# tuanad121/Python-WORLD

Measured on AMD Instinct MI355X. Metric: analysis+synthesis frames/sec (and xRT), 16 kHz / 5 ms hop, higher is better.
Workload: dtype f64; 1 GPU; BASELINE config 2 per GPU: 64 x 10 s synthetic 16 kHz utterances, DIO+StoneMask+CheapTrick+D4C encode + pulse-wise synthesis decode with on-device Philox noise (not the reference-parity host-noise path), HBM-resident; utterances_per_gpu=64, distinct_utterances=64, fs=16000, lanes_per_gpu=1

## Files before the change

python-world_amd/csrc/wh_minphase.h:

```cpp
#pragma once
#include <type_traits>
#include "wh_fft.h"

namespace {

constexpr int ft_syn(int n) { return n >= 2048 ? 512 : 256; }

__device__ __attribute__((noinline)) double4 cis_pair_call(double a0, double b0, double a1, double b1) {
  const double e0 = exp(a0), e1 = exp(a1);
  double s0, c0, s1, c1;
  sincospi(b0, &s0, &c0);
  sincospi(b1, &s1, &c1);
  return make_double4(e0 * c0, e0 * s0, e1 * c1, e1 * s1);
}
__device__ __attribute__((noinline)) double4 cis_pair_tab_call(double a0, double b0, double a1, double b1, wh::ckp<const double2> tw256,
                                                               wh::ckp<const double> mt) {
  const double2 sc0 = wh::tsincospi(b0, tw256), sc1 = wh::tsincospi(b1, tw256);
  const double e0 = wh::texp(a0, mt), e1 = wh::texp(a1, mt);
  return make_double4(e0 * sc0.y, e0 * sc0.x, e1 * sc1.y, e1 * sc1.x);
}
__device__ __attribute__((noinline)) double2 log_pair_call(double x, double y) { return make_double2(wh::flog(x), wh::flog(y)); }
__device__ __attribute__((noinline)) double log_call(double x) { return wh::flog(x); }

template <int M, bool INV, int GT, int FT, bool WAVE>
__device__ __forceinline__ void mp_fft(wh::ckp<double2> zb, wh::ckp<const double2> tw) {
  if constexpr (WAVE) wh::fft_lds_wave<M, INV, GT, FT>(zb, tw);
  else wh::fft_lds<M, INV, GT, FT>(zb, tw);
}
struct SpectrumIdentity {
  __device__ __forceinline__ double2 operator()(int, double2 e) const { return e; }
};
struct NoSide {};
template <int N, int GT, bool WAVE = false, bool TAB = false, class Mul = SpectrumIdentity, class Side = NoSide>
__device__ __forceinline__ void min_phase_response(wh::ckp<double2> zb, wh::ckp<const double2> tw_base, wh::ckp<const double> mt, double delay_pi, Mul mul = Mul(),
                                                   Side side = Side()) {
#pragma clang fp contract(fast)
  constexpr int FT = ft_syn(N);
  constexpr int M = N / 2;
  constexpr int PP = (M / 2 + 1 + GT - 1) / GT;
  const wh::ckp<double> zr = wh::ck_as<double>(zb);
  const int gt = WH_TID & (GT - 1);
  const wh::ckp<const double2> WH_RESTRICT w = tw_base + N;
  if constexpr (WAVE && !std::is_same<Side, NoSide>::value) wh::fft_lds_wave<M, false, GT, FT>(zb, tw_base + M, side);
  else mp_fft<M, false, GT, FT, WAVE>(zb, tw_base + M);
  {
    double ck[PP], cm[PP];
#pragma unroll
    for (int p = 0; p < PP; ++p) {
      const int k = gt + p * GT;
      ck[p] = cm[p] = 0.0;
      if (k <= M / 2) {
        const double2 a = zb[k], b = zb[M - k];
        if (k == 0) {
          ck[p] = a.x + a.y;
          cm[p] = a.x - a.y;
        } else {
          const double er = 0.5 * (a.x + b.x), dr = 0.5 * (a.x - b.x), di = 0.5 * (a.y + b.y);
          const double2 wk = wh::ldg2(w + k);
          const double tr = fma(wk.x, di, wk.y * dr);
          ck[p] = er + tr;
          cm[p] = er - tr;
        }
      }
    }
    wh::sync<FT>();
#pragma unroll
    for (int p = 0; p < PP; ++p) {
      const int k = gt + p * GT;
      if (k <= M / 2) {
        if (k == 0) {
          zr[0] = ck[p];
          zr[M] = 2 * cm[p];
        } else {
          zr[N - k] = 2 * ck[p];
          zr[M + k] = 2 * cm[p];
        }
      }
    }
    for (int n = 1 + gt; n < M; n += GT) zr[n] = 0.0;
    wh::sync<FT>();
  }
  mp_fft<M, false, GT, FT, WAVE>(zb, tw_base + M);
#pragma unroll 1
  for (int k = gt; k <= M / 2; k += GT) {
    const double2 a = zb[k], b = zb[M - k];
    double2 x0, x1;
    const double2 wk = wh::ldg2(w + k);
    if (k == 0) {
      x0 = make_double2(a.x + a.y, 0.0);
      x1 = make_double2(a.x - a.y, 0.0);
    } else {
      const double er = 0.5 * (a.x + b.x), ei = 0.5 * (a.y - b.y);
      const double dr = 0.5 * (a.x - b.x), di = 0.5 * (a.y + b.y);
      const double tr = fma(wk.x, di, wk.y * dr);
      const double ti = fma(wk.y, di, -(wk.x * dr));
      x0 = make_double2(er + tr, ei + ti);
      x1 = make_double2(er - tr, ti - ei);
    }
    const double a0 = x0.x / N, b0 = -x0.y / N * M_1_PI - delay_pi * (double)k;
    const double a1 = x1.x / N, b1 = -x1.y / N * M_1_PI - delay_pi * (double)(M - k);
    double4 cis;
    if constexpr (TAB) cis = cis_pair_tab_call(a0, b0, a1, b1, tw_base + 256, mt);
    else cis = cis_pair_call(a0, b0, a1, b1);
    double2 A = mul(k, make_double2(cis.x, cis.y)), B = mul(M - k, make_double2(cis.z, cis.w));
    if (k == 0) {
      A.y = 0.0;
      B.y = 0.0;
    }
    const double er = A.x + B.x, ei = A.y - B.y;
    const double dr = A.x - B.x, di = A.y + B.y;
    const double orr = fma(dr, wk.x, di * wk.y);
    const double oi = fma(di, wk.x, -(dr * wk.y));
    zb[k] = make_double2(er - oi, ei + orr);
    if (k != 0) zb[M - k] = make_double2(er + oi, orr - ei);
  }
  wh::sync<FT>();
  mp_fft<M, true, GT, FT, WAVE>(zb, tw_base + M);
}

}
```

python-world_amd/csrc/wh_resp_pair.h:

```cpp
#pragma once

namespace {

__device__ __forceinline__ bool resp_pairable(const RespArgs& A, int vuv0, int noise_size0, int vuv1, int noise_size1) {
  const int nd0 = noise_size0 > 3 ? noise_size0 : 3, nd1 = noise_size1 > 3 ? noise_size1 : 3;
  return vuv0 == 0 && vuv1 == 0 && A.noise == nullptr && nd0 + nd1 <= kRespNoise;
}

template <int N>
__device__ __forceinline__ void response_pair(const RespArgs& A, const PulseRec& r0, const PulseRec& r1, char* smem, wh::ckp<double> ring,
                                              RunState& rs, wh::ckp<double> WH_RESTRICT row) {
#pragma clang fp contract(fast)
  const double* __restrict__ spectrogram = A.spectrogram;
  const double2* __restrict__ tw_raw = A.tw_base;
  asm volatile("" : "+s"(tw_raw));
  const wh::ckp<const double2> tw_base = wh::ck_make(tw_raw, WH_TWIDDLE_ENTRIES, wh::WH_CK_TWIDDLE);
  const double* __restrict__ mt_raw = A.math_tab;
  asm volatile("" : "+s"(mt_raw));
  const wh::ckp<const double> mt = wh::ck_make(mt_raw, wh::kMtEntries, wh::WH_CK_TABLE);
  constexpr int FT = ft_syn(N);
  constexpr int K = N / 2 + 1;
  constexpr int NZ = kRespNoise;
  constexpr int R = N / FT;
  constexpr int GT = FT / 2;
  static_assert(GT == 2 * WH_WAVE && R <= 4 && 2 * NZ <= N, "one side wave per chain; the staged noise fits the first chain's buffer");
  using L = RespLds<N>;
  static_assert(NZ == L::kNoiseLen, "the noise block of the layout is the chunk this function stages");
  const wh::ckp<double> lds_all = wh::ck_make(reinterpret_cast<double*>(smem), L::kPulse, wh::WH_CK_LDS_OTHER);
  const wh::ckp<double> zrA = wh::ck_sub(lds_all, L::kChainA, L::kChainLen, wh::WH_CK_LDS_MAIN);
  const wh::ckp<double2> zbA = wh::ck_as<double2>(zrA);
  const wh::ckp<double> zrP = wh::ck_sub(lds_all, L::kChainP, L::kChainLen, wh::WH_CK_LDS_AUX);
  const wh::ckp<double2> zbP = wh::ck_as<double2>(zrP);
  const wh::ckp<double> rap = wh::ck_sub(lds_all, L::kRap, L::kRapLen, wh::WH_CK_LDS_OTHER);
  const wh::ckp<double> nz = wh::ck_sub(lds_all, L::kNoise, L::kNoiseLen, wh::WH_CK_LDS_OTHER);
  const wh::ckp<double> scratch = wh::ck_sub(lds_all, L::kScratch, L::kScratchLen, wh::WH_CK_LDS_SCRATCH);

  RSTAGE_BEGIN
  wh::sync<FT>();
  const int u = r0.u;
  const int64_t ny = A.meta[u].ny;
  RSTAGE_COUNT(kRsNUnvoicedVuv) RSTAGE_COUNT(kRsNUnvoicedVuv) RSTAGE_COUNT(kRsNPairs) RSTAGE_COUNT(kRsNPulses) RSTAGE_COUNT(kRsNPulses)
  {
    const bool same_rows = r0.rows == r1.rows;
    const double* s_lo0 = spectrogram + (r0.rows & 0xffffffffll) * K;
    const double* s_hi0 = spectrogram + (r0.rows >> 32) * K;
    const double* s_lo1 = spectrogram + (r1.rows & 0xffffffffll) * K;
    const double* s_hi1 = spectrogram + (r1.rows >> 32) * K;
    const bool same0 = r0.weight < 0.0, same1 = r1.weight < 0.0;
    const double b0 = same0 ? 0.0 : r0.weight, b1 = same1 ? 0.0 : r1.weight;
    const double a0 = 1 - b0, a1 = 1 - b1;
    constexpr int KQ = (K + FT - 1) / FT;
    double rl0[KQ], rh0[KQ], rl1[KQ], rh1[KQ];
#pragma unroll
    for (int q = 0; q < KQ; ++q) {
      const int k = WH_TID + q * FT;
      const int kc = k < K ? k : K - 1;
      rl0[q] = s_lo0[kc];
      rh0[q] = s_hi0[kc];
    }
    if (same_rows) {
#pragma unroll
      for (int q = 0; q < KQ; ++q) {
        rl1[q] = rl0[q];
        rh1[q] = rh0[q];
      }
    } else {
#pragma unroll
      for (int q = 0; q < KQ; ++q) {
        const int k = WH_TID + q * FT;
        const int kc = k < K ? k : K - 1;
        rl1[q] = s_lo1[kc];
        rh1[q] = s_hi1[kc];
      }
    }
#pragma unroll
    for (int q = 0; q < KQ; ++q) {
      const int k = WH_TID + q * FT;
      if (k >= K) break;
      double w0 = same0 ? rl0[q] : fma(a0, rl0[q], b0 * rh0[q]);
      double w1 = same1 ? rl1[q] : fma(a1, rl1[q], b1 * rh1[q]);
      if (w0 == 0.0) w0 = 2.220446049250313e-16;
      if (w1 == 0.0) w1 = 2.220446049250313e-16;
      const double2 lg = log_pair_call(fabs(w0), fabs(w1));
      const double l0 = lg.x / 2, l1 = lg.y / 2;
      zrA[k] = l0;
      zrP[k] = l1;
      if (k > 0 && k < N / 2) {
        zrA[N - k] = l0;
        zrP[N - k] = l1;
      }
    }
  }
  RSTAGE_MARK(kRsSetup)
  const int nd0 = r0.noise_size > 3 ? r0.noise_size : 3, nd1 = r1.noise_size > 3 ? r1.noise_size : 3;
  const int64_t noff0 = r0.noff, noff1 = r1.noff;
  const uint64_t seed = A.seed;
  auto noise_side = [&](int i, int) {
    const uint64_t key = philox_key(seed, (uint64_t)u);
    const int lane = i & 63;
    const int p = __builtin_amdgcn_readfirstlane(i - lane) >> 6;
    const int64_t noff = p == 0 ? noff0 : noff1;
    const int nd = p == 0 ? nd0 : nd1, at = p == 0 ? 0 : nd0;
    const int64_t blk0 = noff >> 1, b1 = (noff + nd - 1) >> 1;
    for (int c = 0; blk0 + c <= b1; c += 64) {
      const int64_t blk = blk0 + c + lane;
      double part = 0.0;
      if (blk <= b1) {
        const double2 z = normal_pair(key, (uint64_t)blk);
        const int j = (int)(2 * blk - noff);
        if (j >= 0) {
          part += z.x;
          nz[at + j] = z.x;
        }
        if (j + 1 < nd) {
          part += z.y;
          nz[at + j + 1] = z.y;
        }
      }
      part = wh::wave_sum(part);
      if (lane == 0) scratch[4 * p + (c >> 6)] = part;
    }
  };
  wh::sync<FT>();
  RSTAGE_MARK(kRsNoise)
  {
    const int g = WH_TID / GT;
    min_phase_response<N, GT, true, resp_table_cis<N>()>(g == 0 ? zbA : zbP, tw_base, mt, 0.0, SpectrumIdentity(), noise_side);
  }
  RSTAGE_MARK(kRsChainsPair)
  double mean0, mean1;
  {
    const int nb0 = (int)(((noff0 + nd0 - 1) >> 1) - (noff0 >> 1)) + 1, nb1 = (int)(((noff1 + nd1 - 1) >> 1) - (noff1 >> 1)) + 1;
    double t0 = 0.0, t1 = 0.0;
#pragma unroll
    for (int w = 0; w < (NZ / 2 + 1 + 63) / 64; ++w) {
      if (w * 64 < nb0) t0 += scratch[w];
      if (w * 64 < nb1) t1 += scratch[4 + w];
    }
    mean0 = t0 / (double)nd0;
    mean1 = t1 / (double)nd1;
  }
  for (int n = WH_TID; n < N; n += FT) rap[rap_index(n)] = zrA[(n + N / 2) & (N - 1)] / N;
  wh::sync<FT>();
  for (int j = WH_TID; j < NZ; j += FT) {
    zrA[j] = j < nd0 ? nz[j] - mean0 : 0.0;
    zrA[NZ + j] = j < nd1 ? nz[nd0 + j] - mean1 : 0.0;
  }
  wh::sync<FT>();
  const int m0 = WH_TID * R;
  auto excite_and_add = [&](wh::ckp<double> nzb, int nd, int64_t pidx) {
    double acc[R];
#pragma unroll
    for (int q = 0; q < R; ++q) acc[q] = 0.0;
    noise_conv_groups<R>(rap, nzb, nd, m0, 0, acc);
    const int64_t s1 = pidx - N / 2 + 1;
    ring_advance<N>(ring, rs, row, s1, ny);
#pragma unroll
    for (int q = 0; q < R; ++q) {
      const int mm = m0 + q;
      const int64_t tgt = s1 + mm;
      if (tgt < 1) continue;
      if (tgt < ny) ring[(int)(tgt & (N - 1))] += acc[q];
      else if (mm == N - 1) rs.last += acc[q];
    }
  };
  excite_and_add(zrA, nd0, r0.pidx);
  RSTAGE_MARK(kRsConv)
  wh::sync<FT>();
  for (int n = WH_TID; n < N; n += FT) rap[rap_index(n)] = zrP[(n + N / 2) & (N - 1)] / N;
  wh::sync<FT>();
  excite_and_add(zrA + NZ, nd1, r1.pidx);
  RSTAGE_MARK(kRsOverlapAdd)
}

}
```

python-world_amd/csrc/wh_resp_pulse.h:

```cpp
#pragma once

namespace {

template <int R>
__device__ __forceinline__ void noise_conv_groups(wh::ckp<double> rap, wh::ckp<double> nzb, int cnt, int m0, int64_t j0, double (&acc)[R]) {
#pragma clang fp contract(fast)
  auto load_group = [&](int base, double (&g)[R]) {
#pragma unroll
    for (int t = 0; t < R; t += 2) {
      double2 v = make_double2(0.0, 0.0);
      if (base >= 0) v = wh::ck_as<const double2>(rap + rap_index(base + t))[0];
      g[t] = v.x;
      g[t + 1] = v.y;
    }
  };
  auto block = [&](int j, const double (&hi)[R], const double (&lo)[R]) {
    double n[R];
#pragma unroll
    for (int t = 0; t < R; t += 2) {
      const double2 v = wh::ck_as<const double2>(nzb + (j + t))[0];
      n[t] = v.x;
      n[t + 1] = v.y;
    }
#pragma unroll
    for (int sft = 0; sft < R; ++sft)
#pragma unroll
      for (int q = 0; q < R; ++q) acc[q] = fma(n[sft], q - sft >= 0 ? hi[q - sft] : lo[R + q - sft], acc[q]);
  };
  double ga[R], gb[R];
  const int mb0 = m0 - (int)j0;
  load_group(mb0, ga);
  load_group(mb0 - R, gb);
  const int steps = ((cnt + 2 * R - 1) / (2 * R)) * (2 * R);
  for (int j = 0; j < steps; j += 2 * R) {
    block(j, ga, gb);
    load_group(mb0 - j - 2 * R, ga);
    block(j + R, gb, ga);
    load_group(mb0 - j - 3 * R, gb);
  }
}

template <int N>
__device__ __forceinline__ void response_pulse(const RespArgs& A, const PulseRec& rec, char* smem, wh::ckp<double> ring, RunState& rs,
                                               wh::ckp<double> WH_RESTRICT row,
                                               const double (&dcw)[N / ft_syn(N) <= 4 ? N / ft_syn(N) : 1]) {
#pragma clang fp contract(fast)
  const SynUtt* __restrict__ meta = A.meta;
  const double* __restrict__ spectrogram = A.spectrogram;
  const double* __restrict__ aperiodicity = A.aperiodicity;
  const double fs = A.fs;
  const double* __restrict__ noise = A.noise;
  const uint64_t seed = A.seed;
  const double* __restrict__ dc_base = A.dc_base;
  const double2* __restrict__ tw_raw = A.tw_base;
  asm volatile("" : "+s"(tw_raw));
  const wh::ckp<const double2> tw_base = wh::ck_make(tw_raw, WH_TWIDDLE_ENTRIES, wh::WH_CK_TWIDDLE);
  const double* __restrict__ mt_raw = A.math_tab;
  asm volatile("" : "+s"(mt_raw));
  const wh::ckp<const double> mt = wh::ck_make(mt_raw, wh::kMtEntries, wh::WH_CK_TABLE);
  constexpr int FT = ft_syn(N);
  constexpr int K = N / 2 + 1;
  constexpr int NZ = kRespNoise;
  constexpr int NZC = resp_conv8<N>() ? 252 : NZ;
  constexpr int R = N / FT;
  static_assert(R % 2 == 0 && NZ % (2 * R) == 0, "pairwise reads; whole blocks of 2R noise samples");
  constexpr int GT = FT >= 256 ? FT / 2 : FT;
  constexpr int NG = FT / GT;
  using L = RespLds<N>;
  static_assert(NZ == L::kNoiseLen, "the noise block of the layout is the chunk this function stages");
  const wh::ckp<double> lds_all = wh::ck_make(reinterpret_cast<double*>(smem), L::kPulse, wh::WH_CK_LDS_OTHER);
  const wh::ckp<double> zrA = wh::ck_sub(lds_all, L::kChainA, L::kChainLen, wh::WH_CK_LDS_MAIN);
  const wh::ckp<double2> zbA = wh::ck_as<double2>(zrA);
  const wh::ckp<double> zrP = wh::ck_sub(lds_all, L::kChainP, L::kChainLen, wh::WH_CK_LDS_AUX);
  const wh::ckp<double2> zbP = wh::ck_as<double2>(zrP);
  const wh::ckp<double> rap = wh::ck_sub(lds_all, L::kRap, L::kRapLen, wh::WH_CK_LDS_OTHER);
  const wh::ckp<double> nz = wh::ck_sub(lds_all, L::kNoise, L::kNoiseLen, wh::WH_CK_LDS_OTHER);
  const wh::ckp<double> scratch = wh::ck_sub(lds_all, L::kScratch, L::kScratchLen, wh::WH_CK_LDS_SCRATCH);

  RSTAGE_BEGIN
  wh::sync<FT>();
  const int u = rec.u;
  const SynUtt m = meta[u];
  const int64_t pidx = rec.pidx;
  const double shift = rec.shift;
  const int64_t noise_size = rec.noise_size;

  const int64_t row_lo = rec.rows & 0xffffffffll, row_hi = rec.rows >> 32;
  const double bw = rec.weight;
  const bool same = bw < 0.0;
  const double b = same ? 0.0 : bw;
  const double a = 1 - b;
  const double* s_lo = spectrogram + row_lo * K;
  const double* s_hi = spectrogram + row_hi * K;
  const double* a_lo = aperiodicity + row_lo * K;
  const double* a_hi = aperiodicity + row_hi * K;
  constexpr int KQ = (K + FT - 1) / FT;
  double rsl[KQ], rsh[KQ], ral[KQ], rah[KQ];
  const bool need_ap = rec.vuv != 0;
#pragma unroll
  for (int q = 0; q < KQ; ++q) {
    const int k = WH_TID + q * FT;
    const int kc = k < K ? k : K - 1;
    rsl[q] = s_lo[kc];
    rsh[q] = s_hi[kc];
    if constexpr (resp_skip_ap<N>()) {
      ral[q] = rah[q] = 0.0;
    } else {
      ral[q] = a_lo[kc];
      rah[q] = a_hi[kc];
    }
  }
  double ap0_lo, ap0_hi;
  if constexpr (resp_skip_ap<N>()) {
    ap0_lo = ap0_hi = 0.0;
    if (need_ap) {
#pragma unroll
      for (int q = 0; q < KQ; ++q) {
        const int k = WH_TID + q * FT;
        const int kc = k < K ? k : K - 1;
        ral[q] = a_lo[kc];
        rah[q] = a_hi[kc];
      }
      ap0_lo = a_lo[0];
      ap0_hi = a_hi[0];
    }
  } else {
    ap0_lo = a_lo[0];
    ap0_hi = a_hi[0];
  }
  asm volatile("" : "+v"(ap0_lo), "+v"(ap0_hi));
  double aper0;
  {
    const double al = ap0_lo * ap0_lo, ah = ap0_hi * ap0_hi;
    aper0 = same ? al : a * al + b * ah;
  }
  const bool voiced = (rec.vuv != 0) && (aper0 <= 0.999);
  RSTAGE_COUNT(voiced ? kRsNVoiced : (rec.vuv == 0 ? kRsNUnvoicedVuv : kRsNUnvoicedRows))
  RSTAGE_COUNT(kRsNPulses)
#pragma unroll
  for (int q = 0; q < KQ; ++q) {
    const int k = WH_TID + q * FT;
    if (k >= K) break;
    const double sl = rsl[q], sh = rsh[q];
    double v, w;
    auto spectra = [&]() {
      double al = ral[q] * ral[q], ah = rah[q] * rah[q];
      if constexpr (resp_skip_ap<N>()) asm volatile("" : "+v"(al), "+v"(ah));
      const double pl = fmax(0.001, 1 - al), ph = fmax(0.001, 1 - ah);
      const double sp = same ? sl : a * sl + b * sh;
      const double pe = same ? pl : a * pl + b * ph;
      const double ap = same ? al : a * al + b * ah;
      v = sp * pe;
      if (v == 0.0) v = 2.220446049250313e-16;
      w = voiced ? sp * ap : sp;
    };
    if constexpr (resp_skip_ap<N>()) {
      v = 0.0;
      w = same ? sl : a * sl + b * sh;
      if (voiced) spectra();
    } else {
      spectra();
    }
    if (w == 0.0) w = 2.220446049250313e-16;
    double2 lg;
    if (voiced) lg = log_pair_call(fabs(w), fabs(v));
    else lg = make_double2(log_call(fabs(w)), 0.0);
    const double lw = lg.x / 2;
    zrA[k] = lw;
    if (k > 0 && k < N / 2) zrA[N - k] = lw;
    if (voiced) {
      const double lv = lg.y / 2;
      zrP[k] = lv;
      if (k > 0 && k < N / 2) zrP[N - k] = lv;
    }
  }
  RSTAGE_MARK(kRsSetup)
  const int64_t nd = noise_size > 3 ? noise_size : 3;
  const int64_t noff = rec.noff;
  auto noise_at = [&](int64_t j) -> double {
    if (noise) {
      const int64_t q = noff + j;
      return q < m.noise_len ? noise[m.noise_off + q] : 0.0;
    }
    return normal_at(philox_key(seed, (uint64_t)u), (uint64_t)(noff + j));
  };
  constexpr bool ROLES = resp_wave_fft<N>();
  static_assert(!ROLES || NZ / 2 + 1 <= FT, "a run that fits nz is at most one Philox block per thread");
  const bool side_noise = ROLES && noise == nullptr && nd <= NZ;
  auto noise_side = [&](int i, int n) {
    if (!side_noise) return;
    const uint64_t key = philox_key(seed, (uint64_t)u);
    const int lane = i & 63;
    const int64_t blk0 = noff >> 1, b1 = (noff + nd - 1) >> 1;
    for (int c = __builtin_amdgcn_readfirstlane(i - lane); blk0 + c <= b1; c += n) {
      const int64_t blk = blk0 + c + lane;
      double part = 0.0;
      if (blk <= b1) {
        const double2 z = normal_pair(key, (uint64_t)blk);
        const int64_t j = 2 * blk - noff;
        if (j >= 0) {
          part += z.x;
          nz[j] = z.x;
        }
        if (j + 1 < nd) {
          part += z.y;
          nz[j + 1] = z.y;
        }
      }
      part = wh::wave_sum(part);
      if (lane == 0) scratch[c >> 6] = part;
    }
  };
  double mean = 0.0;
  if (side_noise) {
    wh::sync<FT>();
  } else {
    double part = 0.0;
    if (noise) {
      for (int64_t j = WH_TID; j < nd; j += FT) {
        const double v = noise_at(j);
        part += v;
        if (j < NZ) nz[j] = v;
      }
    } else {
      const uint64_t key = philox_key(seed, (uint64_t)u);
      const int64_t b1 = (noff + nd - 1) >> 1;
      for (int64_t blk = (noff >> 1) + WH_TID; blk <= b1; blk += FT) {
        const double2 z = normal_pair(key, (uint64_t)blk);
        const int64_t j = 2 * blk - noff;
        if (j >= 0) {
          part += z.x;
          if (j < NZ) nz[j] = z.x;
        }
        if (j + 1 < nd) {
          part += z.y;
          if (j + 1 < NZ) nz[j + 1] = z.y;
        }
      }
    }
    mean = wh::block_sum<FT>(part, scratch) / (double)nd;
  }

  RSTAGE_MARK(kRsNoise)
  const double coef_pi = 2.0 * fs / N;
  if constexpr (ROLES) {
    if (NG == 2 && voiced) {
      const int g = WH_TID / GT;
      min_phase_response<N, GT, true, resp_table_cis<N>()>(g == 0 ? zbA : zbP, tw_base, mt, g == 0 ? 0.0 : coef_pi * shift, SpectrumIdentity(), noise_side);
    } else {
      min_phase_response<N, FT, true, resp_table_cis<N>()>(zbA, tw_base, mt, 0.0, SpectrumIdentity(), noise_side);
      if (voiced) min_phase_response<N, FT, true, resp_table_cis<N>()>(zbP, tw_base, mt, coef_pi * shift);
    }
  } else if (NG == 2 && voiced) {
    const int g = WH_TID / GT;
    min_phase_response<N, GT, false, resp_table_cis<N>()>(g == 0 ? zbA : zbP, tw_base, mt, g == 0 ? 0.0 : coef_pi * shift);
  } else {
    min_phase_response<N, FT, false, resp_table_cis<N>()>(zbA, tw_base, mt, 0.0);
    if (voiced) min_phase_response<N, FT, false, resp_table_cis<N>()>(zbP, tw_base, mt, coef_pi * shift);
  }
  RSTAGE_MARK(voiced ? kRsChainsVoiced : kRsChainsUnvoiced)
  if (side_noise) {
    const int n_blk = (int)(((noff + nd - 1) >> 1) - (noff >> 1)) + 1;
    double t = 0.0;
#pragma unroll
    for (int w = 0; w < (NZ / 2 + 1 + 63) / 64; ++w)
      if (w * 64 < n_blk) t += scratch[w];
    mean = t / (double)nd;
  }
  for (int n = WH_TID; n < N; n += FT) rap[rap_index(n)] = zrA[(n + N / 2) & (N - 1)] / N;
  wh::sync<FT>();

  double acc[R];
#pragma unroll
  for (int q = 0; q < R; ++q) acc[q] = 0.0;
  double acc8[resp_conv8<N>() ? 8 : 1];
#pragma unroll
  for (int q = 0; q < (resp_conv8<N>() ? 8 : 1); ++q) acc8[q] = 0.0;
  const int m0 = WH_TID * R;
  for (int64_t j0 = 0; j0 < nd; j0 += NZC) {
    const int cnt = (int)(nd - j0 < NZC ? nd - j0 : NZC);
    wh::sync<FT>();
    for (int j = WH_TID; j < NZ; j += FT) {
      double v = 0.0;
      if (j < cnt) v = (j0 == 0 ? nz[j] : noise_at(j0 + j)) - mean;
      nz[j] = v;
    }
    wh::sync<FT>();
    if constexpr (resp_conv8<N>()) {
      constexpr int HT = FT / 2;
      const int half_id = WH_TID / HT, t8 = WH_TID - half_id * HT;
      const int c_all = ((cnt + 11) / 12) * 12;
      const int c_mid = ((c_all / 12 + 1) / 2) * 12;
      const int jb = half_id == 0 ? 0 : c_mid, je = half_id == 0 ? c_mid : c_all;
      auto load4 = [&](int base, double (&g)[4]) {
        double2 v0 = make_double2(0.0, 0.0), v1 = make_double2(0.0, 0.0);
        if (base >= 0) {
          v0 = wh::ck_as<const double2>(rap + rap_index(base))[0];
          v1 = wh::ck_as<const double2>(rap + rap_index(base + 2))[0];
        }
        g[0] = v0.x; g[1] = v0.y; g[2] = v1.x; g[3] = v1.y;
      };
      auto block4 = [&](int j, const double (&hi)[4], const double (&mid)[4], const double (&lo)[4]) {
#pragma unroll
        for (int sp = 0; sp < 4; sp += 2) {
          const double2 nn = wh::ck_as<const double2>(nz + (j + sp))[0];
#pragma unroll
          for (int sft = sp; sft < sp + 2; ++sft)
#pragma unroll
            for (int q = 0; q < 8; ++q) {
              const int idx = q - sft;
              acc8[q] = fma(sft == sp ? nn.x : nn.y, idx >= 4 ? hi[idx - 4] : (idx >= 0 ? mid[idx] : lo[idx + 4]), acc8[q]);
            }
        }
      };
      const int mb0 = t8 * 8 - (int)j0 - jb;
      double g0[4], g1[4], g2[4];
      load4(mb0 + 4, g0);
      load4(mb0, g1);
      load4(mb0 - 4, g2);
      for (int j = jb; j < je; j += 12) {
        const int mb = t8 * 8 - (int)j0 - j;
        block4(j, g0, g1, g2);
        load4(mb - 8, g0);
        block4(j + 4, g1, g2, g0);
        load4(mb - 12, g1);
        block4(j + 8, g2, g0, g1);
        load4(mb - 16, g2);
      }
    } else if constexpr (R <= 4) {
      auto load_group = [&](int base, double (&g)[R]) {
  #pragma unroll
        for (int t = 0; t < R; t += 2) {
          double2 v = make_double2(0.0, 0.0);
          if (base >= 0) v = wh::ck_as<const double2>(rap + rap_index(base + t))[0];
          g[t] = v.x;
          g[t + 1] = v.y;
        }
      };
      auto block = [&](int j, const double (&hi)[R], const double (&lo)[R]) {
        double n[R];
  #pragma unroll
        for (int t = 0; t < R; t += 2) {
          const double2 v = wh::ck_as<const double2>(nz + (j + t))[0];
          n[t] = v.x;
          n[t + 1] = v.y;
        }
  #pragma unroll
        for (int sft = 0; sft < R; ++sft)
  #pragma unroll
          for (int q = 0; q < R; ++q) acc[q] = fma(n[sft], q - sft >= 0 ? hi[q - sft] : lo[R + q - sft], acc[q]);
      };
      double ga[R], gb[R];
      const int mb0 = m0 - (int)j0;
      load_group(mb0, ga);
      load_group(mb0 - R, gb);
      const int steps = ((cnt + 2 * R - 1) / (2 * R)) * (2 * R);
      for (int j = 0; j < steps; j += 2 * R) {
        block(j, ga, gb);
        load_group(mb0 - j - 2 * R, ga);
        block(j + R, gb, ga);
        load_group(mb0 - j - 3 * R, gb);
      }
    } else {
      double r[R];
  #pragma unroll
      for (int q = 0; q < R; ++q) {
        const int idx = m0 + q - (int)j0;
        r[q] = idx >= 0 ? rap[rap_index(idx)] : 0.0;
      }
      const int steps = (cnt + 1) & ~1;
      for (int j = 0; j < steps; j += 2) {
        const double2 nn = wh::ck_as<const double2>(nz + j)[0];
        const int inew = m0 - (int)j0 - j - 2;
        double2 fresh = make_double2(0.0, 0.0);
        if (inew >= 0) fresh = wh::ck_as<const double2>(rap + rap_index(inew))[0];
  #pragma unroll
        for (int q = 0; q < R; ++q) acc[q] = fma(nn.x, r[q], acc[q]);
  #pragma unroll
        for (int q = R - 1; q > 0; --q) r[q] = r[q - 1];
        r[0] = fresh.y;
  #pragma unroll
        for (int q = 0; q < R; ++q) acc[q] = fma(nn.y, r[q], acc[q]);
  #pragma unroll
        for (int q = R - 1; q > 0; --q) r[q] = r[q - 1];
        r[0] = fresh.x;
      }
    }
  }

  if constexpr (resp_conv8<N>()) {
    constexpr int HT = FT / 2;
    const int half_id = WH_TID / HT, t8 = WH_TID - half_id * HT;
    wh::sync<FT>();
    const wh::ckp<double> park = half_id == 0 ? zrA : rap;
#pragma unroll
    for (int q = 0; q < 8; q += 2) wh::ck_as<double2>(park + (t8 * 8 + q))[0] = make_double2(acc8[q], acc8[q + 1]);
    wh::sync<FT>();
#pragma unroll
    for (int q = 0; q < R; q += 2) {
      const double2 a = wh::ck_as<const double2>(zrA + (m0 + q))[0], b2 = wh::ck_as<const double2>(rap + (m0 + q))[0];
      acc[q] = a.x + b2.x;
      acc[q + 1] = a.y + b2.y;
    }
  }
  RSTAGE_MARK(kRsConv)
  double dc_total = 0.0;
  const double gain = sqrt((double)(noise_size > 1 ? noise_size : 1));
  if (voiced) {
    double part = 0.0;
    for (int n = WH_TID; n < N; n += FT) part += zrP[n] / N;
    dc_total = wh::block_sum<FT>(part, scratch);
  }

  const int64_t s1 = pidx - N / 2 + 1;
  ring_advance<N>(ring, rs, row, s1, m.ny);
#pragma unroll
  for (int q = 0; q < R; ++q) {
    const int mm = m0 + q;
    const int64_t tgt = s1 + mm;
    double v = acc[q];
    if (voiced) v += (zrP[(mm + N / 2) & (N - 1)] / N + (R <= 4 && !resp_conv8<N>() ? dcw[R <= 4 ? q : 0] : dc_base[mm]) * -dc_total) * gain;
    if (tgt < 1) continue;
    if (tgt < m.ny) ring[(int)(tgt & (N - 1))] += v;
    else if (mm == N - 1) rs.last += v;
  }
  RSTAGE_MARK(kRsOverlapAdd)
}

}
```

python-world_amd/csrc/wh_resp_ring.h:

```cpp
#pragma once

namespace {

template <int N>
__device__ __forceinline__ void ring_flush(wh::ckp<double> ring, int64_t a, int64_t b, wh::ckp<double> WH_RESTRICT row, int64_t row_start,
                                           int64_t ny) {
  constexpr int FT = ft_syn(N);
  a = a < 1 ? 1 : a;
  b = b > ny ? ny : b;
  for (int64_t tgt = a + WH_TID; tgt < b; tgt += FT) {
    const int slot = (int)(tgt & (N - 1));
    row[1 + (tgt - row_start)] = ring[slot];
    ring[slot] = 0.0;
  }
}

template <int N>
__device__ __forceinline__ void ring_advance(wh::ckp<double> ring, RunState& rs, wh::ckp<double> WH_RESTRICT row, int64_t s1, int64_t ny) {
  constexpr int FT = ft_syn(N);
  if (rs.any) {
    const int64_t e = s1 < rs.win_start + N ? s1 : rs.win_start + N;
    ring_flush<N>(ring, rs.win_start, e, row, rs.row_start, ny);
    for (int64_t tgt = rs.win_start + N + WH_TID; tgt < (s1 < ny ? s1 : ny); tgt += FT) row[1 + (tgt - rs.row_start)] = 0.0;
    wh::sync<FT>();
  } else {
    rs.row_start = s1 < 1 ? 1 : s1;
  }
  rs.any = true;
  rs.win_start = s1;
}

}
```

python-world_amd/csrc/wh_resp_types.h:

```cpp
#pragma once
#include "wh_minphase.h"

enum RespStage {
  kRsNoise = 0,
  kRsChainsVoiced = 2,
  kRsConv = 3,
  kRsOverlapAdd = 4,
  kRsSetup = 5,
  kRsChainsUnvoiced = 6,
  kRsChainsPair = 7,
  kRsNVoiced = 8,
  kRsNUnvoicedVuv = 9,
  kRsNUnvoicedRows = 10,
  kRsNPartner = 11,
  kRsNPairs = 12,
  kRsNPulses = 13
};
#ifdef WH_RESP_STAGE_TIMER
static __device__ unsigned long long g_resp_stage[16];
#define RSTAGE_BEGIN unsigned long long _t0 = __builtin_readcyclecounter();
#define RSTAGE_MARK(i) { __syncthreads(); if (threadIdx.x == 0) { const unsigned long long _t = __builtin_readcyclecounter(); atomicAdd(&g_resp_stage[i], _t - _t0); _t0 = _t; } }
#define RSTAGE_COUNT(i) { if (threadIdx.x == 0) atomicAdd(&g_resp_stage[i], 1ull); }
#else
#define RSTAGE_BEGIN
#define RSTAGE_MARK(i)
#define RSTAGE_COUNT(i)
#endif

namespace {
using wh::SynUtt;
using wh::PulseRec;

template <int N>
constexpr bool resp_conv8() { return N / ft_syn(N) == 4 && N >= 2048; }

template <int N>
constexpr bool resp_wave_fft() { return N == 1024; }
template <int N>
constexpr bool resp_skip_ap() { return resp_wave_fft<N>(); }
template <int N>
constexpr bool resp_pairs() { return resp_wave_fft<N>() && ft_syn(N) == 256; }

template <int N>
constexpr bool resp_table_cis() { return N >= 1024; }

constexpr int resp_run(int n) { return n <= 1024 ? 6 : 8; }

__device__ __forceinline__ int rap_index(int i) { return i + 2 * (i >> 5); }

constexpr int kRespNoise = 256;
template <int N>
struct RespLds {
  static constexpr int kChainLen = N + 2;
  static constexpr int kChainA = 0;
  static constexpr int kChainP = kChainA + kChainLen;
  static constexpr int kRap = kChainP + kChainLen;
  static constexpr int kRapLen = N + N / 16 + 2;
  static constexpr int kNoise = kRap + kRapLen;
  static constexpr int kNoiseLen = kRespNoise;
  static constexpr int kScratch = kNoise + kNoiseLen;
  static constexpr int kScratchLen = 32;
  static constexpr int kPulse = kScratch + kScratchLen;
  static constexpr int kRing = kPulse;
  static constexpr int kRingLen = N;
  static constexpr int kTotal = kRing + kRingLen;
};

struct RespArgs {
  const SynUtt* meta;
  const double* tp;
  const double* spectrogram;
  const double* aperiodicity;
  double fs;
  const PulseRec* p_rec;
  const int64_t* p_base;
  int n_utt;
  const double* noise;
  uint64_t seed;
  const double* dc_base;
  const double2* tw_base;
  const double* math_tab;
  double* rows;
  const int64_t* row_base;
  const int64_t* run_base;
  const int64_t* row_off;
  int64_t runs_cap;
};

struct RunState {
  bool any;
  int64_t win_start;
  int64_t row_start;
  double last;
};

}
```

python-world_amd/csrc/wh_synthesis.hip:

```cpp
#include "wh_host.h"
#include "wh_tid.h"
#include "wh_device.h"
#include "wh_math.h"
#include "wh_reduce.h"
#include "wh_syn_types.h"
#include "wh_minphase.h"
#include "wh_philox.h"
#include "wh_resp_types.h"
#include "wh_resp_ring.h"
#include "wh_resp_pulse.h"
#include "wh_resp_pair.h"

namespace {
using wh::block_excl_scan_256;
using wh::first_pulse_at;

__global__ __launch_bounds__(256) void philox_dump_kernel(uint64_t seed, int32_t u, int64_t q0, int64_t n,
                                                          double* __restrict__ out) {
  const int64_t i = (int64_t)blockIdx.x * 256 + threadIdx.x;
  if (i < n) out[i] = normal_at(philox_key(seed, (uint64_t)u), (uint64_t)(q0 + i));
}
__global__ __launch_bounds__(64) void noise_cover_kernel(const SynUtt* __restrict__ meta, const PulseRec* __restrict__ rec,
                                                         const int64_t* __restrict__ p_base, int n_utt,
                                                         int32_t* __restrict__ flags) {
// ... 209 lines not shown
  if (n0 + kGatherTile >= m.ny) {
    const int k_end = first_pulse_at(pi, count, m.ny - N / 2);
    if (threadIdx.x == 0) {
      double last = 0.0;
      for (int r = k_end / RUN; r < n_runs; ++r) {
        const int64_t off = ro[r];
        if (off >= 0) last += ru[off];
      }
      y[m.y_off + m.ny - 1] = last;
    }
  }
}

struct RespCall {
  int B;
  int64_t pcap_max, max_ny;
  const std::vector<int64_t>* h_ny;
  const SynUtt* d_meta;
  const double* tp;
  const double* spec;
  const double* ap;
  double fs;
  const PulseRec* p_rec;
  const int64_t* p_base;
  const int64_t* p_idx;
  const int32_t* p_count;
  const double* noise;
  uint64_t seed;
  double* y;
};

template <int N>
int launch_resp(wh_ctx* ctx, hipStream_t st, const RespCall& c) {
  const int B = c.B;
  const int64_t pcap_max = c.pcap_max, max_ny = c.max_ny;
  const std::vector<int64_t>& h_ny = *c.h_ny;
  const SynUtt* d_meta = c.d_meta;
  const int64_t* p_idx = c.p_idx;
  const int32_t* p_count = c.p_count;
  std::vector<double> dc(N);
  double sum = 0.0;
  for (int n = 0; n < N; ++n) {
    dc[n] = 0.5 - 0.5 * cos(2.0 * M_PI * (double)(n + 1) / (double)(N + 1));
    sum += dc[n];
  }
  for (int n = 0; n < N; ++n) dc[n] /= sum;
  const double* d_dc = nullptr;
  if (int rc = wh::const_table(ctx, "dc_base:" + std::to_string(N), dc, &d_dc)) return rc;
  const double* d_mt = nullptr;
  if (int rc = wh::math_table(ctx, &d_mt)) return rc;
  const size_t lds = sizeof(double) * RespLds<N>::kTotal;
  if (int rc = wh::allow_lds(&response_kernel<N>, lds)) return rc;
  const int64_t runs_cap = (pcap_max + resp_run(N) - 1) / resp_run(N);
  int64_t per_sample = (96 * pcap_max + max_ny - 1) / (max_ny > 0 ? max_ny : 1);
  per_sample = per_sample < 12 ? 12 : (per_sample > 48 ? 48 : per_sample);
  std::vector<int64_t> row_base((size_t)B + 1, 0);
  for (int u = 0; u < B; ++u) row_base[u + 1] = row_base[u] + per_sample * h_ny[u] + 4 * (N + 1);
  int64_t* d_row_base = nullptr;
  if (int rc = wh::persistent_upload(ctx, st, "syn.row_base", row_base, &d_row_base)) return rc;
  double* d_rows = nullptr;
  int64_t *d_rb = nullptr, *d_ro = nullptr;
  if (int rc = wh::persistent_scratch(ctx, "syn.ola_rows", (size_t)row_base[B], &d_rows)) return rc;
  if (int rc = wh::persistent_scratch(ctx, "syn.run_base", (size_t)B + 1, &d_rb)) return rc;
  if (int rc = wh::persistent_scratch(ctx, "syn.row_off", (size_t)runs_cap * B, &d_ro)) return rc;
  WH_LAUNCH(ctx, st, "pulse_run_base_kernel", pulse_run_base_kernel, dim3(1), dim3(64), 0, p_count, B, resp_run(N), d_rb);
  WH_LAUNCH(ctx, st, "pulse_rows_kernel", pulse_rows_kernel<N>, dim3(B), dim3(256), 0, d_meta, p_idx, p_count, runs_cap,
            d_row_base, d_ro, ctx->d_flags);
  const int64_t grid = wh::xcd_grid(runs_cap * B);
  const RespArgs ra{d_meta, c.tp, c.spec, c.ap, c.fs, c.p_rec, c.p_base, B, c.noise, c.seed, d_dc, ctx->d_twiddle, d_mt,
                    d_rows, d_row_base, d_rb, d_ro, runs_cap};
  WH_LAUNCH(ctx, st, "response_kernel", response_kernel<N>, dim3((unsigned)grid), dim3(ft_syn(N)), lds, ra);
  WH_LAUNCH(ctx, st, "response_gather_kernel", response_gather_kernel<N>,
            dim3((unsigned)((max_ny + kGatherTile - 1) / kGatherTile), B), dim3(256), 0, d_meta, p_idx, p_count,
            d_rows, d_row_base, d_ro, runs_cap, c.y);
  return 0;
}

}

extern "C" int wh_synthesis_render(wh_ctx* ctx, void* stream, const wh_batch* b, const wh_ctx* timebase_ctx,
                                   const double* tp, const double* spectrogram, const double* aperiodicity, double fs,
                                   int fft_size, const int64_t* h_y_off, const double* h_t0, const double* h_dt,
                                   int64_t pulse_cap, const double* noise, const int64_t* h_noise_off, uint64_t seed,
                                   double* y, int32_t* pulse_count_out) {
  if (!ctx || !b || !timebase_ctx || !tp || !spectrogram || !aperiodicity || !h_y_off || !h_t0 || !h_dt || !y)
    return wh::fail_msg("wh_synthesis_render", "null argument");
  WH_ENTER(ctx);
  if (noise && !h_noise_off) return wh::fail_msg("wh_synthesis_render", "noise given without h_noise_off");
  hipStream_t st = (hipStream_t)stream;
  const int B = b->n_utt;
  const wh_ctx::TimeBase& t = timebase_ctx->timebase;
  if (!t.valid || t.n_utt != B || t.pulse_cap != pulse_cap || t.ny_tot != h_y_off[B] || t.frames != b->total_frames ||
      timebase_ctx->device != ctx->device)
    return wh::fail_msg("wh_synthesis_render", "no matching time base in timebase_ctx (run wh_synthesis_timebase on it "
                                               "with the same batch, lengths and pulse_cap, and nothing else since)");
  std::vector<SynUtt> meta;
  int64_t max_ny = 0;
  if (int rc = wh::fill_syn_meta("wh_synthesis_render", b, h_y_off, h_t0, h_dt, pulse_cap, noise, h_noise_off, meta, &max_ny)) return rc;
  const void* ws = timebase_ctx->ws;
  SynUtt* d_meta = nullptr;
  if (int rc = wh::persistent_upload(ctx, st, "syn.meta", meta, &d_meta)) return rc;
  const int64_t* d_pb = t.pb.at(ws);
  const int64_t* d_pi = t.pi.at(ws);
  const PulseRec* d_rec = t.rec.at(ws);
  const int32_t* d_pc = t.pc.at(ws);
  if (noise)
    WH_LAUNCH(ctx, st, "noise_cover_kernel", noise_cover_kernel, dim3((unsigned)((B + 63) / 64)), dim3(64), 0, d_meta,
              d_rec, d_pb, B, ctx->d_flags);
  std::vector<int64_t> h_ny((size_t)B);
  for (int u = 0; u < B; ++u) h_ny[u] = meta[u].ny;
  const RespCall call{B, pulse_cap, max_ny, &h_ny, d_meta, tp, spectrogram, aperiodicity, fs, d_rec, d_pb, d_pi, d_pc, noise, seed, y};
  int rc = 0;
  if (!wh::dispatch_fft_size(fft_size, [&](auto n) { rc = launch_resp<decltype(n)::value>(ctx, st, call); }))
    return wh::fail_msg("wh_synthesis_render", "fft_size must be a power of two in [512, 4096]");
  if (rc) return rc;
  if (pulse_count_out) WH_CHECK(hipMemcpyAsync(pulse_count_out, d_pc, sizeof(int32_t) * B, hipMemcpyDeviceToDevice, st));
  return 0;
}

extern "C" int wh_synthesis(wh_ctx* ctx, void* stream, const wh_batch* b, const double* tp, const double* f0,
                            const double* vuv, const double* spectrogram, const double* aperiodicity, double fs,
                            int fft_size, const int64_t* h_y_off, const double* h_t0, const double* h_dt,
                            int64_t pulse_cap, const double* noise, const int64_t* h_noise_off, uint64_t seed, double* y,
                            int32_t* pulse_count_out) {
  if (!ctx || !b || !tp || !f0 || !vuv || !spectrogram || !aperiodicity || !h_y_off || !h_t0 || !h_dt || !y)
    return wh::fail_msg("wh_synthesis", "null argument");
  if (noise && !h_noise_off) return wh::fail_msg("wh_synthesis", "noise given without h_noise_off");
  if (!wh::dispatch_fft_size(fft_size, [](auto) {}))
    return wh::fail_msg("wh_synthesis", "fft_size must be a power of two in [512, 4096]");
  if (int rc = wh_synthesis_timebase(ctx, stream, b, tp, f0, vuv, fs, h_y_off, h_t0, h_dt, pulse_cap, 0.0)) return rc;
  return wh_synthesis_render(ctx, stream, b, ctx, tp, spectrogram, aperiodicity, fs, fft_size, h_y_off, h_t0, h_dt, pulse_cap,
                             noise, h_noise_off, seed, y, pulse_count_out);
}

extern "C" int wh_philox_normals(wh_ctx* ctx, void* stream, uint64_t seed, int utt, int64_t q0, int64_t n, double* out) {
  if (!ctx || !out || utt < 0 || q0 < 0 || n < 0) return wh::fail_msg("wh_philox_normals", "bad argument");
  WH_ENTER(ctx);
  if (n == 0) return 0;
  hipStream_t st = (hipStream_t)stream;
  WH_LAUNCH(ctx, st, "philox_dump_kernel", philox_dump_kernel, dim3((unsigned)((n + 255) / 256)), dim3(256), 0, seed,
            (int32_t)utt, q0, n, out);
  return 0;
}

#ifdef WH_RESP_STAGE_TIMER
extern "C" int wh_debug_resp_stages(unsigned long long* out16, int reset) {
  (void)hipMemcpyFromSymbol(out16, HIP_SYMBOL(g_resp_stage), sizeof(unsigned long long) * 16);
  if (reset) {
    unsigned long long z[16] = {0};
    (void)hipMemcpyToSymbol(HIP_SYMBOL(g_resp_stage), z, sizeof(z));
  }
  return 0;
}
#endif
```

Measured before the change: 14.95 million frames/s.

## Overlap noise staging and ring advance with min-phase FFTs via side-wave callbacks

Extends min_phase_response so that each of its three FFTs can run a side-wave callback, and uses them to do noise mean-subtraction and staging during the second FFT and the ring-buffer advance during the third. The serial tail passes and barriers that used to follow the chains are dropped. In the role-split path the voiced DC sum is captured from the spectrum at k=0 through a multiplier tap, replacing a block reduction. This adds padding of the noise to whole blocks of 2R, changes the LDS noise layout, and adds optional stage-timer instrumentation, at the cost of more complex code and added register pressure inside the FFT.

```diff
diff --git a/python-world_amd/csrc/wh_minphase.h b/python-world_amd/csrc/wh_minphase.h
--- a/python-world_amd/csrc/wh_minphase.h
+++ b/python-world_amd/csrc/wh_minphase.h
@@ -31,9 +31,15 @@
   __device__ __forceinline__ double2 operator()(int, double2 e) const { return e; }
 };
 struct NoSide {};
-template <int N, int GT, bool WAVE = false, bool TAB = false, class Mul = SpectrumIdentity, class Side = NoSide>
+template <int M, bool INV, int GT, int FT, bool WAVE, class Side>
+__device__ __forceinline__ void mp_fft(wh::ckp<double2> zb, wh::ckp<const double2> tw, Side side) {
+  if constexpr (WAVE && !std::is_same<Side, NoSide>::value) wh::fft_lds_wave<M, INV, GT, FT>(zb, tw, side);
+  else mp_fft<M, INV, GT, FT, WAVE>(zb, tw);
+}
+template <int N, int GT, bool WAVE = false, bool TAB = false, class Mul = SpectrumIdentity, class Side = NoSide, class Side2 = NoSide,
+          class Side3 = NoSide>
 __device__ __forceinline__ void min_phase_response(wh::ckp<double2> zb, wh::ckp<const double2> tw_base, wh::ckp<const double> mt, double delay_pi, Mul mul = Mul(),
-                                                   Side side = Side()) {
+                                                   Side side = Side(), Side2 side2 = Side2(), Side3 side3 = Side3()) {
 #pragma clang fp contract(fast)
   constexpr int FT = ft_syn(N);
   constexpr int M = N / 2;
@@ -41,8 +47,7 @@
   const wh::ckp<double> zr = wh::ck_as<double>(zb);
   const int gt = WH_TID & (GT - 1);
   const wh::ckp<const double2> WH_RESTRICT w = tw_base + N;
-  if constexpr (WAVE && !std::is_same<Side, NoSide>::value) wh::fft_lds_wave<M, false, GT, FT>(zb, tw_base + M, side);
-  else mp_fft<M, false, GT, FT, WAVE>(zb, tw_base + M);
+  mp_fft<M, false, GT, FT, WAVE>(zb, tw_base + M, side);
   {
     double ck[PP], cm[PP];
 #pragma unroll
@@ -80,7 +85,7 @@
     for (int n = 1 + gt; n < M; n += GT) zr[n] = 0.0;
     wh::sync<FT>();
   }
-  mp_fft<M, false, GT, FT, WAVE>(zb, tw_base + M);
+  mp_fft<M, false, GT, FT, WAVE>(zb, tw_base + M, side2);
 #pragma unroll 1
   for (int k = gt; k <= M / 2; k += GT) {
     const double2 a = zb[k], b = zb[M - k];
@@ -115,7 +120,7 @@
     if (k != 0) zb[M - k] = make_double2(er + oi, orr - ei);
   }
   wh::sync<FT>();
-  mp_fft<M, true, GT, FT, WAVE>(zb, tw_base + M);
+  mp_fft<M, true, GT, FT, WAVE>(zb, tw_base + M, side3);
 }
 
 }
diff --git a/python-world_amd/csrc/wh_resp_pair.h b/python-world_amd/csrc/wh_resp_pair.h
--- a/python-world_amd/csrc/wh_resp_pair.h
+++ b/python-world_amd/csrc/wh_resp_pair.h
@@ -23,9 +23,9 @@
   constexpr int NZ = kRespNoise;
   constexpr int R = N / FT;
   constexpr int GT = FT / 2;
-  static_assert(GT == 2 * WH_WAVE && R <= 4 && 2 * NZ <= N, "one side wave per chain; the staged noise fits the first chain's buffer");
+  static_assert(GT == 2 * WH_WAVE && R <= 4, "one side wave per chain");
   using L = RespLds<N>;
-  static_assert(NZ == L::kNoiseLen, "the noise block of the layout is the chunk this function stages");
+  static_assert(NZ + 4 * R <= L::kNoiseLen, "two runs of NZ samples together, each zero-padded to whole blocks of 2R");
   const wh::ckp<double> lds_all = wh::ck_make(reinterpret_cast<double*>(smem), L::kPulse, wh::WH_CK_LDS_OTHER);
   const wh::ckp<double> zrA = wh::ck_sub(lds_all, L::kChainA, L::kChainLen, wh::WH_CK_LDS_MAIN);
   const wh::ckp<double2> zbA = wh::ck_as<double2>(zrA);
@@ -93,6 +93,7 @@
   }
   RSTAGE_MARK(kRsSetup)
   const int nd0 = r0.noise_size > 3 ? r0.noise_size : 3, nd1 = r1.noise_size > 3 ? r1.noise_size : 3;
+  const int pad0 = ((nd0 + 2 * R - 1) / (2 * R)) * (2 * R), pad1 = ((nd1 + 2 * R - 1) / (2 * R)) * (2 * R);
   const int64_t noff0 = r0.noff, noff1 = r1.noff;
   const uint64_t seed = A.seed;
   auto noise_side = [&](int i, int) {
@@ -100,7 +101,7 @@
     const int lane = i & 63;
     const int p = __builtin_amdgcn_readfirstlane(i - lane) >> 6;
     const int64_t noff = p == 0 ? noff0 : noff1;
-    const int nd = p == 0 ? nd0 : nd1, at = p == 0 ? 0 : nd0;
+    const int nd = p == 0 ? nd0 : nd1, at = p == 0 ? 0 : pad0;
     const int64_t blk0 = noff >> 1, b1 = (noff + nd - 1) >> 1;
     for (int c = 0; blk0 + c <= b1; c += 64) {
       const int64_t blk = blk0 + c + lane;
@@ -121,40 +122,42 @@
       if (lane == 0) scratch[4 * p + (c >> 6)] = part;
     }
   };
+  auto stage_side = [&](int i, int) {
+    const int lane = i & 63;
+    const int p = __builtin_amdgcn_readfirstlane(i - lane) >> 6;
+    const int64_t noff = p == 0 ? noff0 : noff1;
+    const int nd = p == 0 ? nd0 : nd1, at = p == 0 ? 0 : pad0, pad = p == 0 ? pad0 : pad1;
+    const int nb = (int)(((noff + nd - 1) >> 1) - (noff >> 1)) + 1;
+    double t = 0.0;
+#pragma unroll
+    for (int w = 0; w < (NZ / 2 + 1 + 63) / 64; ++w)
+      if (w * 64 < nb) t += scratch[4 * p + w];
+    const double mean = t / (double)nd;
+    for (int j = lane; j < pad; j += 64) nz[at + j] = j < nd ? nz[at + j] - mean : 0.0;
+  };
+  const int64_t s1_0 = r0.pidx - N / 2 + 1;
+  auto ring_side = [&](int i, int n) { ring_advance_side<N>(ring, rs, row, s1_0, ny, i, n); };
   wh::sync<FT>();
   RSTAGE_MARK(kRsNoise)
   {
     const int g = WH_TID / GT;
-    min_phase_response<N, GT, true, resp_table_cis<N>()>(g == 0 ? zbA : zbP, tw_base, mt, 0.0, SpectrumIdentity(), noise_side);
+    min_phase_response<N, GT, true, resp_table_cis<N>()>(g == 0 ? zbA : zbP, tw_base, mt, 0.0, SpectrumIdentity(), noise_side, stage_side, ring_side);
   }
+  ring_advance_done(rs, s1_0);
   RSTAGE_MARK(kRsChainsPair)
-  double mean0, mean1;
-  {
-    const int nb0 = (int)(((noff0 + nd0 - 1) >> 1) - (noff0 >> 1)) + 1, nb1 = (int)(((noff1 + nd1 - 1) >> 1) - (noff1 >> 1)) + 1;
-    double t0 = 0.0, t1 = 0.0;
-#pragma unroll
-    for (int w = 0; w < (NZ / 2 + 1 + 63) / 64; ++w) {
-      if (w * 64 < nb0) t0 += scratch[w];
-      if (w * 64 < nb1) t1 += scratch[4 + w];
-    }
-    mean0 = t0 / (double)nd0;
-    mean1 = t1 / (double)nd1;
-  }
   for (int n = WH_TID; n < N; n += FT) rap[rap_index(n)] = zrA[(n + N / 2) & (N - 1)] / N;
   wh::sync<FT>();
-  for (int j = WH_TID; j < NZ; j += FT) {
-    zrA[j] = j < nd0 ? nz[j] - mean0 : 0.0;
-    zrA[NZ + j] = j < nd1 ? nz[nd0 + j] - mean1 : 0.0;
-  }
-  wh::sync<FT>();
+  RSTAGE_TAIL(kRtPair, kRtCopy)
   const int m0 = WH_TID * R;
-  auto excite_and_add = [&](wh::ckp<double> nzb, int nd, int64_t pidx) {
+  auto excite_and_add = [&](wh::ckp<double> nzb, int nd, int64_t pidx, bool advance) {
     double acc[R];
 #pragma unroll
     for (int q = 0; q < R; ++q) acc[q] = 0.0;
     noise_conv_groups<R>(rap, nzb, nd, m0, 0, acc);
+    RSTAGE_TAIL(kRtPair, kRtConv)
     const int64_t s1 = pidx - N / 2 + 1;
-    ring_advance<N>(ring, rs, row, s1, ny);
+    if (advance) ring_advance<N>(ring, rs, row, s1, ny);
+    RSTAGE_TAIL(kRtPair, kRtAdvance)
 #pragma unroll
     for (int q = 0; q < R; ++q) {
       const int mm = m0 + q;
@@ -163,13 +166,15 @@
       if (tgt < ny) ring[(int)(tgt & (N - 1))] += acc[q];
       else if (mm == N - 1) rs.last += acc[q];
     }
+    RSTAGE_TAIL(kRtPair, kRtAdd)
   };
-  excite_and_add(zrA, nd0, r0.pidx);
+  excite_and_add(nz, nd0, r0.pidx, false);
   RSTAGE_MARK(kRsConv)
   wh::sync<FT>();
   for (int n = WH_TID; n < N; n += FT) rap[rap_index(n)] = zrP[(n + N / 2) & (N - 1)] / N;
   wh::sync<FT>();
-  excite_and_add(zrA + NZ, nd1, r1.pidx);
+  RSTAGE_TAIL(kRtPair, kRtCopy)
+  excite_and_add(nz + pad0, nd1, r1.pidx, true);
   RSTAGE_MARK(kRsOverlapAdd)
 }
 
diff --git a/python-world_amd/csrc/wh_resp_pulse.h b/python-world_amd/csrc/wh_resp_pulse.h
--- a/python-world_amd/csrc/wh_resp_pulse.h
+++ b/python-world_amd/csrc/wh_resp_pulse.h
@@ -39,6 +39,16 @@
     load_group(mb0 - j - 3 * R, gb);
   }
 }
+
+struct SpectrumDcTap {
+  wh::ckp<double> slot;
+  bool on;
+  __device__ __forceinline__ double2 operator()(int k, double2 e) const {
+    if (on && k == 0) slot[0] = e.x;
+    return e;
+  }
+};
+constexpr int kDcSlot = 31;
 
 template <int N>
 __device__ __forceinline__ void response_pulse(const RespArgs& A, const PulseRec& rec, char* smem, wh::ckp<double> ring, RunState& rs,
@@ -67,7 +77,7 @@
   constexpr int GT = FT >= 256 ? FT / 2 : FT;
   constexpr int NG = FT / GT;
   using L = RespLds<N>;
-  static_assert(NZ == L::kNoiseLen, "the noise block of the layout is the chunk this function stages");
+  static_assert(NZ <= L::kNoiseLen, "the noise block of the layout holds the chunk this function stages");
   const wh::ckp<double> lds_all = wh::ck_make(reinterpret_cast<double*>(smem), L::kPulse, wh::WH_CK_LDS_OTHER);
   const wh::ckp<double> zrA = wh::ck_sub(lds_all, L::kChainA, L::kChainLen, wh::WH_CK_LDS_MAIN);
   const wh::ckp<double2> zbA = wh::ck_as<double2>(zrA);
@@ -211,6 +221,19 @@
       if (lane == 0) scratch[c >> 6] = part;
     }
   };
+  auto stage_side = [&](int i, int n) {
+    if (!side_noise) return;
+    const int n_blk = (int)(((noff + nd - 1) >> 1) - (noff >> 1)) + 1;
+    double t = 0.0;
+#pragma unroll
+    for (int w = 0; w < (NZ / 2 + 1 + 63) / 64; ++w)
+      if (w * 64 < n_blk) t += scratch[w];
+    const double mean_s = t / (double)nd;
+    const int cnt = (int)nd, pad = ((cnt + 2 * R - 1) / (2 * R)) * (2 * R);
+    for (int j = i; j < pad; j += n) nz[j] = j < cnt ? nz[j] - mean_s : 0.0;
+  };
+  const int64_t s1 = pidx - N / 2 + 1;
+  auto ring_side = [&](int i, int n) { ring_advance_side<N>(ring, rs, row, s1, m.ny, i, n); };
   double mean = 0.0;
   if (side_noise) {
     wh::sync<FT>();
@@ -246,11 +269,13 @@
   if constexpr (ROLES) {
     if (NG == 2 && voiced) {
       const int g = WH_TID / GT;
-      min_phase_response<N, GT, true, resp_table_cis<N>()>(g == 0 ? zbA : zbP, tw_base, mt, g == 0 ? 0.0 : coef_pi * shift, SpectrumIdentity(), noise_side);
-    } else {
-      min_phase_response<N, FT, true, resp_table_cis<N>()>(zbA, tw_base, mt, 0.0, SpectrumIdentity(), noise_side);
-      if (voiced) min_phase_response<N, FT, true, resp_table_cis<N>()>(zbP, tw_base, mt, coef_pi * shift);
-    }
+      min_phase_response<N, GT, true, resp_table_cis<N>()>(g == 0 ? zbA : zbP, tw_base, mt, g == 0 ? 0.0 : coef_pi * shift,
+                                                           SpectrumDcTap{scratch + kDcSlot, g != 0}, noise_side, stage_side, ring_side);
+    } else {
+      static_assert(NG == 2, "the single chain of this branch is an unvoiced pulse's");
+      min_phase_response<N, FT, true, resp_table_cis<N>()>(zbA, tw_base, mt, 0.0, SpectrumIdentity(), noise_side, stage_side, ring_side);
+    }
+    ring_advance_done(rs, s1);
   } else if (NG == 2 && voiced) {
     const int g = WH_TID / GT;
     min_phase_response<N, GT, false, resp_table_cis<N>()>(g == 0 ? zbA : zbP, tw_base, mt, g == 0 ? 0.0 : coef_pi * shift);
@@ -259,16 +284,9 @@
     if (voiced) min_phase_response<N, FT, false, resp_table_cis<N>()>(zbP, tw_base, mt, coef_pi * shift);
   }
   RSTAGE_MARK(voiced ? kRsChainsVoiced : kRsChainsUnvoiced)
-  if (side_noise) {
-    const int n_blk = (int)(((noff + nd - 1) >> 1) - (noff >> 1)) + 1;
-    double t = 0.0;
-#pragma unroll
-    for (int w = 0; w < (NZ / 2 + 1 + 63) / 64; ++w)
-      if (w * 64 < n_blk) t += scratch[w];
-    mean = t / (double)nd;
-  }
   for (int n = WH_TID; n < N; n += FT) rap[rap_index(n)] = zrA[(n + N / 2) & (N - 1)] / N;
   wh::sync<FT>();
+  RSTAGE_TAIL(voiced ? kRtVoiced : kRtSingle, kRtCopy)
 
   double acc[R];
 #pragma unroll
@@ -279,13 +297,16 @@
   const int m0 = WH_TID * R;
   for (int64_t j0 = 0; j0 < nd; j0 += NZC) {
     const int cnt = (int)(nd - j0 < NZC ? nd - j0 : NZC);
-    wh::sync<FT>();
-    for (int j = WH_TID; j < NZ; j += FT) {
-      double v = 0.0;
-      if (j < cnt) v = (j0 == 0 ? nz[j] : noise_at(j0 + j)) - mean;
-      nz[j] = v;
-    }
-    wh::sync<FT>();
+    if (!side_noise) {
+      wh::sync<FT>();
+      for (int j = WH_TID; j < NZ; j += FT) {
+        double v = 0.0;
+        if (j < cnt) v = (j0 == 0 ? nz[j] : noise_at(j0 + j)) - mean;
+        nz[j] = v;
+      }
+      wh::sync<FT>();
+      RSTAGE_TAIL(voiced ? kRtVoiced : kRtSingle, kRtStage)
+    }
     if constexpr (resp_conv8<N>()) {
       constexpr int HT = FT / 2;
       const int half_id = WH_TID / HT, t8 = WH_TID - half_id * HT;
@@ -403,17 +424,23 @@
       acc[q + 1] = a.y + b2.y;
     }
   }
+  RSTAGE_TAIL(voiced ? kRtVoiced : kRtSingle, kRtConv)
   RSTAGE_MARK(kRsConv)
   double dc_total = 0.0;
   const double gain = sqrt((double)(noise_size > 1 ? noise_size : 1));
   if (voiced) {
-    double part = 0.0;
-    for (int n = WH_TID; n < N; n += FT) part += zrP[n] / N;
-    dc_total = wh::block_sum<FT>(part, scratch);
-  }
-
-  const int64_t s1 = pidx - N / 2 + 1;
-  ring_advance<N>(ring, rs, row, s1, m.ny);
+    if constexpr (ROLES) {
+      dc_total = scratch[kDcSlot];
+    } else {
+      double part = 0.0;
+      for (int n = WH_TID; n < N; n += FT) part += zrP[n] / N;
+      dc_total = wh::block_sum<FT>(part, scratch);
+    }
+  }
+  RSTAGE_TAIL(voiced ? kRtVoiced : kRtSingle, kRtDcSum)
+
+  if constexpr (!ROLES) ring_advance<N>(ring, rs, row, s1, m.ny);
+  RSTAGE_TAIL(voiced ? kRtVoiced : kRtSingle, kRtAdvance)
 #pragma unroll
   for (int q = 0; q < R; ++q) {
     const int mm = m0 + q;
@@ -424,6 +451,7 @@
     if (tgt < m.ny) ring[(int)(tgt & (N - 1))] += v;
     else if (mm == N - 1) rs.last += v;
   }
+  RSTAGE_TAIL(voiced ? kRtVoiced : kRtSingle, kRtAdd)
   RSTAGE_MARK(kRsOverlapAdd)
 }
 
diff --git a/python-world_amd/csrc/wh_resp_ring.h b/python-world_amd/csrc/wh_resp_ring.h
--- a/python-world_amd/csrc/wh_resp_ring.h
+++ b/python-world_amd/csrc/wh_resp_ring.h
@@ -30,4 +30,23 @@
   rs.win_start = s1;
 }
 
+template <int N>
+__device__ __forceinline__ void ring_advance_side(wh::ckp<double> ring, const RunState& rs, wh::ckp<double> WH_RESTRICT row, int64_t s1, int64_t ny,
+                                                  int i, int n) {
+  if (!rs.any) return;
+  const int64_t e = s1 < rs.win_start + N ? s1 : rs.win_start + N;
+  const int64_t a = rs.win_start < 1 ? 1 : rs.win_start, b = e > ny ? ny : e;
+  for (int64_t tgt = a + i; tgt < b; tgt += n) {
+    const int slot = (int)(tgt & (N - 1));
+    row[1 + (tgt - rs.row_start)] = ring[slot];
+    ring[slot] = 0.0;
+  }
+  for (int64_t tgt = rs.win_start + N + i; tgt < (s1 < ny ? s1 : ny); tgt += n) row[1 + (tgt - rs.row_start)] = 0.0;
 }
+__device__ __forceinline__ void ring_advance_done(RunState& rs, int64_t s1) {
+  if (!rs.any) rs.row_start = s1 < 1 ? 1 : s1;
+  rs.any = true;
+  rs.win_start = s1;
+}
+
+}
diff --git a/python-world_amd/csrc/wh_resp_types.h b/python-world_amd/csrc/wh_resp_types.h
--- a/python-world_amd/csrc/wh_resp_types.h
+++ b/python-world_amd/csrc/wh_resp_types.h
@@ -16,14 +16,26 @@
   kRsNPairs = 12,
   kRsNPulses = 13
 };
+enum RespTailKind { kRtVoiced = 0, kRtSingle = 1, kRtPair = 2 };
+enum RespTailPart {
+  kRtCopy = 0,
+  kRtStage = 1,
+  kRtConv = 2,
+  kRtDcSum = 3,
+  kRtAdvance = 4,
+  kRtAdd = 5
+};
 #ifdef WH_RESP_STAGE_TIMER
 static __device__ unsigned long long g_resp_stage[16];
-#define RSTAGE_BEGIN unsigned long long _t0 = __builtin_readcyclecounter();
-#define RSTAGE_MARK(i) { __syncthreads(); if (threadIdx.x == 0) { const unsigned long long _t = __builtin_readcyclecounter(); atomicAdd(&g_resp_stage[i], _t - _t0); _t0 = _t; } }
+static __device__ unsigned long long g_resp_tail[32];
+#define RSTAGE_BEGIN unsigned long long _t0 = __builtin_readcyclecounter(), _t1 = _t0;
+#define RSTAGE_MARK(i) { __syncthreads(); if (threadIdx.x == 0) { const unsigned long long _t = __builtin_readcyclecounter(); atomicAdd(&g_resp_stage[i], _t - _t0); _t0 = _t1 = _t; } }
+#define RSTAGE_TAIL(kind, part) { __syncthreads(); if (threadIdx.x == 0) { const unsigned long long _t = __builtin_readcyclecounter(); atomicAdd(&g_resp_tail[(kind) * 8 + (part)], _t - _t1); _t1 = _t; } }
 #define RSTAGE_COUNT(i) { if (threadIdx.x == 0) atomicAdd(&g_resp_stage[i], 1ull); }
 #else
 #define RSTAGE_BEGIN
 #define RSTAGE_MARK(i)
+#define RSTAGE_TAIL(kind, part)
 #define RSTAGE_COUNT(i)
 #endif
 
@@ -57,7 +69,7 @@
   static constexpr int kRap = kChainP + kChainLen;
   static constexpr int kRapLen = N + N / 16 + 2;
   static constexpr int kNoise = kRap + kRapLen;
-  static constexpr int kNoiseLen = kRespNoise;
+  static constexpr int kNoiseLen = kRespNoise + (resp_pairs<N>() ? 16 : 0);
   static constexpr int kScratch = kNoise + kNoiseLen;
   static constexpr int kScratchLen = 32;
   static constexpr int kPulse = kScratch + kScratchLen;
diff --git a/python-world_amd/csrc/wh_synthesis.hip b/python-world_amd/csrc/wh_synthesis.hip
--- a/python-world_amd/csrc/wh_synthesis.hip
+++ b/python-world_amd/csrc/wh_synthesis.hip
@@ -385,4 +385,12 @@
   }
   return 0;
 }
+extern "C" int wh_debug_resp_tail(unsigned long long* out32, int reset) {
+  (void)hipMemcpyFromSymbol(out32, HIP_SYMBOL(g_resp_tail), sizeof(unsigned long long) * 32);
+  if (reset) {
+    unsigned long long z[32] = {0};
+    (void)hipMemcpyToSymbol(HIP_SYMBOL(g_resp_tail), z, sizeof(z));
+  }
+  return 0;
+}
 #endif
```

New measurement: 15.09 million frames/s (median of 6 runs). No clear change (+0.9%).
